# ztlpn/minilp

Measured on AMD Instinct MI355X. Metric: simplex pivots/sec, higher is better.
Workload: dtype f64; 1 GPU; config 4: random LP 100000 vars x 100000 constraints, 100 nnz/row (0.1% fill), Max c'x, Ax<=b, x>=0; primal simplex with PSE+DSE from the slack basis; timed pivots 5..1983; parallelism=1 GPU, nucleus_size_at_end=1559, completed_steps=1978

## Files before the change

minilp_amd/csrc/engine.h:

```cpp
#pragma once
#include <hip/hip_runtime.h>

#include <cstdint>
#include <functional>
#include <utility>
#include <stdexcept>
#include <string>
#include <vector>

#include "kernels.h"

namespace mlp {

enum Stage { STAGE_FTRAN = 0, STAGE_RATIO = 1, STAGE_BTRAN = 2, STAGE_BASIS = 3, STAGE_ROW = 4, STAGE_APPLY = 5 };

struct MlpError : std::runtime_error {
    int code;
    MlpError(int c, const std::string& s) : std::runtime_error(s), code(c) {}
};
struct LpFail {
    int code;
};

#define HIPCHECK(expr)                                                                                   \
// ... 109 lines not shown
    double fold_bytes = 0, fold_ms = 0;
    uint64_t fold_launches = 0;
    uint64_t kase[5] = {0, 0, 0, 0, 0};
};

enum class IterForm : int { Plain, PrimalHead, SmallBasis, MediumRide, LargeRide, ShardedPull, Factor };
enum class FtranEntry : int { Fused, GatherLrh, PrepGather };
enum class RowForm : int { Inside, Sparse, Sweep };
struct IterPlan {
    int phase, pse, dse, lazy, wtau, inl, fac;
    IterForm form;
    FtranEntry ftran;
    int ftran_ys, ftran_fpk;
    int tk_ride, rk_inside;
    int v_ride;
    int btran, btran_rhs;
    int sb_tk_inside;
    int post_touch, post_rk_ride;
    int basis_lists_touched;
    RowForm row;
    int row_lists;
    int pull_inside, with_struct;
    int fac_fused, fac_rho_part, fac_pair;
};

class Engine {
public:
    Engine();
    ~Engine();
    Engine(const Engine&) = delete;
// ... 420 lines not shown
```

minilp_amd/csrc/engine.hip:

```cpp
#include "engine.h"


#include <algorithm>
#include <chrono>
#include <cmath>
#include <cstdio>
#include <cstdlib>
#include <climits>
#include <cstring>
#include <limits>
#include <map>
#include <memory>
#include <mutex>

#include <dlfcn.h>
#include <fcntl.h>
#include <sys/mman.h>
#include <sys/stat.h>
#include <unistd.h>

namespace mlp {

static const double INF = std::numeric_limits<double>::infinity();
static double now_s() {
// ... 1310 lines not shown
    const bool fpl_base = g.fp && phase == 0 && pse && lazy && !stepping && !smallb && !g.head_fused && max_col_nnz_ <= HEAD_LIST_CAP && fpull_supported(dv, g);
    const bool fpl = fpl_base && ((tkr && ftran_head_rides_gather(dv, g)) || (shard_world > 1 && dv.lrJ > 0 && dv.pb_on && !dv.det_pull && dv.rowinfo != nullptr));
    const bool btr = !phead && !smallb && !tkr && !fpl && phase == 0 && pse && lazy && !stepping && shard_world == 1 && !shard_is_live() && btran_rides_ratio(dv, g);
    pl.form = phead ? IterForm::PrimalHead : smallb ? IterForm::SmallBasis : btr ? IterForm::MediumRide : tkr ? IterForm::LargeRide
              : fpl ? IterForm::ShardedPull : IterForm::Plain;
    if (phase == 0 && g.head_fused) pl.ftran = FtranEntry::Fused;
    else if (phase == 0 && !stepping && max_col_nnz_ <= HEAD_LIST_CAP && (fpl || ftran_head_rides_gather(dv, g))) pl.ftran = FtranEntry::GatherLrh;
    else pl.ftran = FtranEntry::PrepGather;
    pl.ftran_ys = tkr ? 1 : 0, pl.ftran_fpk = fpl ? 1 : 0;
    pl.tk_ride = tkr ? 1 : ((tkr_s || btr) ? 2 : 0), pl.rk_inside = btr ? 1 : 0;
    pl.btran = (phead || smallb || rkr || btr) ? 0 : 1;
    pl.btran_rhs = (phase == 0 && !tkr && !fpl) ? pse : 0;
    pl.sb_tk_inside = tkr_s ? 0 : 1;
    pl.post_touch = (g.str && phase == 0) ? 1 : 0, pl.post_rk_ride = rkr ? 1 : 0;
    pl.v_ride = (btr && !pl.post_touch && v_rides_ratio(dv, g)) ? 1 : 0;
    pl.basis_lists_touched = (phead || smallb || post_fused_lists_touched(dv, g, pse, 0, pl.post_touch)) ? 1 : 0;
    pl.pull_inside = (phead && g.str && update_pulls_inside(dv, g)) ? (head_applies(dv, g) ? 2 : 1) : 0;
    pl.row = !g.str ? RowForm::Sweep : (pl.pull_inside ? RowForm::Inside : RowForm::Sparse);
    pl.row_lists = (phase == 1 && !g.str && sweep_lists(dv, 0, 1)) ? 1 : 0;
    pl.with_struct = (phase == 1 && !pse) ? 1 : 0;
    return pl;
}
void Engine::launch_stage(const IterPlan& pl, int stage, bool with_events) {
    const DevView& dv = hview;
    const Geom g = geom();
    const int phase = pl.phase, pse = pl.pse;
    const bool phead = pl.form == IterForm::PrimalHead;
    if (phead && (stage == STAGE_RATIO || stage == STAGE_BTRAN || stage == STAGE_BASIS)) return;
    const bool fused = pl.fac_fused, pair = pl.fac_pair;
    const int dse = pl.dse, rho_whole = pl.fac_rho_part ? 0 : 8;
// ... 50 lines not shown
        break;
    case STAGE_BASIS:
        if (pl.fac) {
            if (pse && !(phase == 0 && pair)) launch_fac_solve(dv, g, 1, 1, 1, nullptr, 0, st);
            if (dse && !(phase == 1 && pair)) launch_fac_solve(dv, g, 0, 1, 1, nullptr, 0, st);
            break;
        }
        if (pl.form == IterForm::SmallBasis) {
            time_slot(2, 2);
            launch_small_basis(dv, g, st, pl.sb_tk_inside);
            time_slot(2, -1);
            break;
        }
        if (pl.v_ride) {
            time_slot(2, 2);
            launch_eta_vtail(dv, g, st);
            time_slot(2, -1);
            break;
        }
        time_slot(2, 2), time_slot(3, 10);
        launch_fused_w(dv, g, pse, st, pl.wtau);
        time_slot(2, -1), time_slot(3, -1);
        launch_post_fused(dv, g, pse, st, 0, 0, pl.wtau, pl.post_touch, pl.post_rk_ride);
        break;
    case STAGE_ROW:
        if (pl.row == RowForm::Inside) stamp(0), stamp(1);
        else if (pl.row == RowForm::Sparse) {
            stamp(0);
            if (phase == 0) launch_row_sparse(dv, g, pse, phead ? 0 : 1, pl.basis_lists_touched ? 0 : 1, st);
            else launch_row_sparse(dv, g, 0, 0, 1, st);
            stamp(1);
        } else {
            if (!pl.fac) time_slot(1, 0);
            if (phase == 0) launch_sweep(dv, g, pse, pl.fac ? 0 : 1, st, pl.inl);
            else launch_sweep(dv, g, 0, 0, st, 0, 1);
            if (!pl.fac) time_slot(1, -1);
        }
        break;
    case STAGE_APPLY:
        if (phase == 1 && pse) {
            if (pl.row == RowForm::Sparse) launch_row_sparse(dv, g, 2, 1, 0, st);
            else launch_sweep(dv, g, 2, pl.fac ? 0 : 1, st);
        }
        stamp(4);
        if (pl.fac && !fused) launch_fac_append(dv, st);
        launch_update_pivot(dv, g, phase, dse, pse, st, pl.inl, pl.with_struct, pl.pull_inside);
        stamp(5);
        break;
    default:
        throw MlpError(-1, "unknown stage");
    }
}
static bool use_graph_env() {
    const char* ng = std::getenv("MLP_NO_GRAPH");
    return !(ng && ng[0] == '1');
}
void Engine::record_iteration(const IterPlan& pl, bool with_events) {
    if (with_events) HIPCHECK(hipEventRecord(ev[8], st));
    static const bool debug_sync = std::getenv("MLP_DEBUG_SYNC") != nullptr && !use_graph_env();
    for (int i = 0; i < 6; ++i) {
        launch_stage(pl, kStageOrder[pl.phase][i], with_events);
// ... 1834 lines not shown
        tmp = {(double)n_, (double)p_};
    } else if (w == "fpull") {
        tmp = {(double)(hview.fpk_on ? 1 : 0), (double)fpk_builds_, (double)fpk_built_at_, (double)(fpull_supported(hview, geom()) ? 1 : 0)};
    } else if (w == "ratio_primal_form") {
        tmp = {(double)ratio_primal_form(hview, geom())};
    } else if (w == "ratio_list") {
        pull_ctl();
        const Geom g_ = geom();
        tmp = {(double)((ratio_primal_form(hview, g_) == 1 && ratio_list_cap(hview, g_) >= 0) ? 1 : 0), (double)h_ctl->rl_decisions, (double)h_ctl->rl_overflows};
    } else if (w == "btran_ride") {
        pull_ctl();
        tmp = {(double)(btran_rides_ratio(hview, geom()) ? 1 : 0), (double)h_ctl->rk_rides};
    } else if (w == "v_ride") {
        pull_ctl();
        tmp = {(double)(v_rides_ratio(hview, geom()) ? 1 : 0), (double)h_ctl->v_rides};
    } else if (w == "golive_checks") {
        tmp = {(double)golive_checks_};
    } else if (w == "shard_live") {
        tmp = {(double)(shard_is_live() ? 1 : 0)};
    } else if (w == "primal_head_launches") {
        pull_ctl();
        tmp = {(double)h_ctl->ph_count};
    }
    else if (w == "hyper_profile") {
        pull_ctl();
        for (int i = 0; i < 13; ++i) tmp.push_back((double)h_ctl->hy_prof[i] * 0.01);
        tmp.push_back((double)h_ctl->hy_prof[13]);
        tmp.push_back((double)h_ctl->hy_prof[14] * 0.01);
        tmp.push_back(0.0);
        for (int i = 16; i < 24; ++i) tmp.push_back((double)h_ctl->hy_prof[i] * 0.01);
// ... 945 lines not shown
```

minilp_amd/csrc/kernels.h:

```cpp
#pragma once
#include <hip/hip_runtime.h>
#include <stdint.h>

namespace mlp {

constexpr double EPS = 1e-8;

enum IterStatus : int {
    ITER_PIVOT = 0,
    ITER_FLIP = 1,
    ITER_OPTIMAL = 2,
    ITER_UNBOUNDED = 3,
    ITER_FEASIBLE = 4,
    ITER_INFEASIBLE = 5,
    ITER_SINGULAR = 6,
    ITER_NONE = 7,
    ITER_COMM = 8,
    ITER_STALL = 9,
};

struct IterState {
    int status;
    int q;
    int r;
// ... 66 lines not shown
    int ph_count;
    int ph_rng_x, ph_rng_y;
    int ar_used;
    int ar_n;
    int rv_n;
    unsigned long long hy_prof[24];
    PivotRec ring[RING];
    int ar_off;
    int ar_back;
    int ar_pauses;
    int ar_keep;
    int rk_rides;
    int rl_decisions;
    int rl_overflows;
    int v_rides;
};

constexpr int MAIL_KINDS = 6;
constexpr int MAX_WORLD = 16;
struct alignas(64) MailRec {
    unsigned long long epoch;
    double f[7];
};

constexpr uint8_t NB_AT_MIN = 1, NB_AT_MAX = 2, NB_FIXED = 4;
__host__ __device__ inline int nb_status_of(uint8_t f) {
    if ((f & NB_FIXED) || ((f & NB_AT_MIN) && (f & NB_AT_MAX))) return 4;
    return (f & NB_AT_MIN) ? 1 : ((f & NB_AT_MAX) ? 2 : 3);
}

// ... 165 lines not shown
    int* fac_brow;
    int* fac_bslot_of_row;
    double* fac_Wb;
    const FacSbRec* fac_sb_rec; const int* fac_sb_lptr; const int* fac_sb_oidx; const double* fac_sb_oval;
    const int* fac_sb_trow; const int* fac_sb_tcol; const double* fac_sb_tinv; const double* fac_sb_tinvT;
};
constexpr int FAC_BMAX = 1024;
constexpr int AR_CAP = 2048;
constexpr int RK_LDS = 64;
constexpr int RL_CAP = 8;
constexpr int RL_BLOCKS = 512;
constexpr int TK_ONE = 128;
constexpr int TK_GROUPS = 16;
constexpr int TK_STRIDE = 1024;
constexpr int TK_WORDS = TK_STRIDE * (TK_GROUPS + 1) + 8;
constexpr int FAC_BAR_FLAG = TK_WORDS + 1024;

constexpr int FW_TR = 8;
constexpr int FW_TC = 1024;

constexpr int BAND_ROWS = 8192;
constexpr int BAND_THREADS = 1024;
constexpr int PB_ROWS = 4096;
constexpr int PB_CHUNKS = 48;
constexpr int PB_CHUNKS_DEFAULT = 24;

struct Geom {
    int m, n, cap;
    int lanes;
    int sweep_one;
// ... 17 lines not shown
void launch_price_dual(const DevView& dv, const Geom& g, int use_dse, hipStream_t st);
void launch_ftran_prep(const DevView& dv, int derive_primal, hipStream_t st);
void launch_ftran_gather(const DevView& dv, const Geom& g, hipStream_t st, int ys = 0);
void launch_ftran_fused(const DevView& dv, const Geom& g, int derive_primal, hipStream_t st);
bool ftran_head_rides_gather(const DevView& dv, const Geom& g);
void launch_ftran_gather_lrh(const DevView& dv, const Geom& g, hipStream_t st, int ys = 0, int fpk = 0);
bool fpull_supported(const DevView& dv, const Geom& g);
void launch_fpull_ratio(const DevView& dv, const Geom& g, hipStream_t st, hipEvent_t ftran_done = nullptr);
void launch_fpk_build(const DevView& dv, hipStream_t st);
void launch_btran_fused(const DevView& dv, const Geom& g, int with_rhs, int derive_dual, hipStream_t st);
constexpr int HEAD_LIST_CAP = 1024;
void launch_ratio_primal(const DevView& dv, const Geom& g, int use_pse, hipStream_t st, int tk_ride = 0, int rk_inside = 0, int v_ride = 0);
bool tk_rides_ratio(const DevView& dv, const Geom& g);
bool btran_rides_ratio(const DevView& dv, const Geom& g);
bool v_rides_ratio(const DevView& dv, const Geom& g);
void launch_eta_vtail(const DevView& dv, const Geom& g, hipStream_t st);
int ratio_list_cap(const DevView& dv, const Geom& g);
int ratio_primal_form(const DevView& dv, const Geom& g);
bool tk_rides_ratio_small(const DevView& dv, const Geom& g);
void launch_post_ftran(const DevView& dv, const Geom& g, int use_pse, hipStream_t st);
void launch_btran_prep(const DevView& dv, int derive_dual, int plan_after, hipStream_t st);
void launch_btran(const DevView& dv, const Geom& g, int with_rhs, hipStream_t st, int after_fold = 0);
void launch_btran_rhs(const DevView& dv, const Geom& g, hipStream_t st);
void launch_sweep(const DevView& dv, const Geom& g, int mode, int with_struct, hipStream_t st, int inline_combine = 0, int list = 0);
void launch_row_sparse(const DevView& dv, const Geom& g, int mode, int with_struct, int touch, hipStream_t st);
bool small_basis_supported(const DevView& dv, const Geom& g);
void launch_small_basis(const DevView& dv, const Geom& g, hipStream_t st, int tk_inside = 1);
bool primal_head_supported(const DevView& dv, const Geom& g);
int primal_head_kmax(int longest_column);
void launch_primal_head(const DevView& dv, hipStream_t st, int list, int applies);
void launch_init_nb_rng(const DevView& dv, const Geom& g, hipStream_t st);
void launch_ratio_dual(const DevView& dv, const Geom& g, hipStream_t st, int list_ok = 0);
void launch_fused_w(const DevView& dv, const Geom& g, int with_v, hipStream_t st, int with_tau = 1);
void launch_post_fused(const DevView& dv, const Geom& g, int with_v, hipStream_t st, int classic = 0, int skip_push = 0, int with_tau = 1, int touch = 0, int rk_ride = 0);
bool rk_rides_post(const DevView& dv, const Geom& g);
void launch_exact_beta(const DevView& dv, hipStream_t st);
void launch_hyper_dual(const DevView& dv, int use_dse, int max_iters, long heavy, hipStream_t st);
void launch_mail_handshake(const DevView& dv, int* out, hipStream_t st);
constexpr int MAIL_PUMP_RECS = MAIL_KINDS * 2 + 1;
void launch_mail_stage(const DevView& dv, void* stage, hipStream_t st);
void launch_mail_deliver(const DevView& dv, const void* stage, hipStream_t st);
void arm_kernel_timing(int slot, hipEvent_t t0, hipEvent_t t1);
bool fold_fuses_v(const DevView& dv, int with_v, int with_tau, int fold_only);
int stream_coresident_blocks();
void launch_structure_update(const DevView& dv, const Geom& g, hipStream_t st);
void launch_update_pivot(const DevView& dv, const Geom& g, int phase, int use_dse, int use_pse, hipStream_t st, int inline_comb = 0,
                         int with_struct = 0, int pull_inside = 0);
bool update_pulls_inside(const DevView& dv, const Geom& g);
bool head_applies(const DevView& dv, const Geom& g);
void launch_set_iter(const DevView& dv, int status, int q, int r, double lnv, int forced, hipStream_t st);
void launch_reset_ring(const DevView& dv, hipStream_t st);
void launch_btran_dense(const DevView& dv, const Geom& g, hipStream_t st);
void launch_recalc_d(const DevView& dv, const Geom& g, hipStream_t st);
void launch_recalc_basic_vals(const DevView& dv, const Geom& g, const double* rhs, double* r_tmp, int refine, hipStream_t st);
void launch_shift_nonbasic(const DevView& dv, const Geom& g, int col, double val, hipStream_t st);
void launch_sq_norms_add_row(const DevView& dv, const Geom& g, hipStream_t st);
void launch_copy_rho_sq_to_beta(const DevView& dv, int row, hipStream_t st);
void launch_build_nucleus(const DevView& dv, const Geom& g, double* Kd, int k, hipStream_t st);
void launch_fac_solve(const DevView& dv, const Geom& g, int dir, int src, int dst, const double* src_ptr, int always, hipStream_t st, int fuse = 0);
void launch_fac_solve2(const DevView& dv, const Geom& g, int dir, int srcA, int dstA, int srcB, int dstB, hipStream_t st, int fuse = 0);
void fac_solve_set_sharers(int n);
int fac_solve_grid_blocks();
// ... 159 lines not shown
```

minilp_amd/csrc/kernels.hip:

```cpp
#include "kernels.h"
#include <hip/hip_ext.h>

#include <limits.h>
#include <math.h>

#include <cstdlib>
#include <string>

namespace mlp {

#define NONE_IDX INT_MAX
constexpr int BLK = 256;

struct Cand {
    double key;
    int idx;
};
__device__ __forceinline__ Cand cand_none() { return Cand{-INFINITY, NONE_IDX}; }
__device__ __forceinline__ bool cand_better(const Cand& a, const Cand& b) {
    return a.key > b.key || (a.key == b.key && a.idx < b.idx);
}
__device__ __forceinline__ Cand wave_best(Cand c) {
#pragma unroll
    for (int o = 32; o > 0; o >>= 1) {
// ... 157 lines not shown
        s_key[w] = c.key;
        s_idx[w] = c.idx;
        s_pay[w] = pay;
    }
    __syncthreads();
    if (threadIdx.x == 0) {
        for (int i = 1; i < BLK / 64; ++i) {
            Cand t{s_key[i], s_idx[i]};
            if (cand_better(t, c)) {
                c = t;
                pay = s_pay[i];
            }
        }
    }
}
__device__ __forceinline__ bool grid_best_p(Cand& c, double& pay, const DevView& v, int nblocks = -1) {
    if (nblocks < 0) nblocks = (int)gridDim.x;
    block_best_p(c, pay);
    if (threadIdx.x == 0) {
        st_agent(&v.red_key[blockIdx.x], c.key);
        st_agent(&v.red_idx[blockIdx.x], c.idx);
        st_agent(&v.red_key2[blockIdx.x], pay);
    }
    if (!last_block_arrives(v.ticket, (unsigned)nblocks)) return false;
    KMARK(v.ctl, 16);
    Cand x = cand_none();
    double xp = 0.0;
    for (int i = threadIdx.x; i < nblocks; i += blockDim.x) {
        Cand t{ld_agent(&v.red_key[i]), ld_agent(&v.red_idx[i])};
        if (cand_better(t, x)) {
            x = t;
            xp = ld_agent(&v.red_key2[i]);
        }
    }
    KMARK(v.ctl, 17);
    block_best_p(x, xp);
    c = x;
    pay = xp;
    if (threadIdx.x == 0) *v.ticket = 0;
// ... 47 lines not shown
}
#define LAUNCH_T(slot, kern, grid, block, lds, st, ...)                                                          \
    do {                                                                                                         \
        if (g_tev[slot][0]) hipExtLaunchKernelGGL(kern, grid, block, lds, st, g_tev[slot][0], g_tev[slot][1], 0, __VA_ARGS__); \
        else hipLaunchKernelGGL(kern, grid, block, lds, st, __VA_ARGS__);                                        \
    } while (0)
static inline int blocks_for(long n, int per_block = BLK) { return n <= 0 ? 1 : (int)((n + per_block - 1) / per_block); }

template <int G>
__device__ __forceinline__ double group_sum(double x) {
#pragma unroll
    for (int o = G / 2; o > 0; o >>= 1) x += __shfl_xor(x, o, 64);
    return x;
}

__device__ __forceinline__ void push_rec(Ctl* c, int phase) {
    int n = c->ring_n;
    if (n < RING) {
        PivotRec& r = c->ring[n];
        r.status = c->it.status;
        r.phase = phase;
        r.q = c->it.q;
        r.r = c->it.r;
        r.entering_var = c->it.entering_var;
        r.leaving_var = c->it.leaving_var;
        r.kase = c->up.kase;
        r.k_after = c->k;
        r.klist_n = c->it.klist_n;
        r.blist_n = c->it.blist_n;
        r.pivot_coeff = c->it.pivot_coeff;
        if (c->kprof_on == 2) r.pivot_coeff = c->it.alpha_sq;
        else if (c->kprof_on == 3) r.pivot_coeff = c->it.rho_sq;
        else if (c->kprof_on == 4) r.pivot_coeff = c->it.inv_alpha;
        else if (c->kprof_on == 5) {
            double sh = 0.0;
            for (int j = 0; j < c->nlow && j < LR_MAX; ++j) sh += c->lr_h[j];
            r.pivot_coeff = sh;
        }
        r.obj = c->it.obj;
    }
    c->ring_n = n + 1;
}
// ... 498 lines not shown
        it->q = -1;
        it->r = -1;
        c->halt = 1;
        push_rec(c, phase);
    } else {
        it->status = ITER_PIVOT;
        if (phase == 0) {
            it->q = best.idx;
            it->r = -1;
        } else {
            it->r = best.idx;
            it->q = -1;
        }
    }
}
__device__ __forceinline__ void close_and_open(const DevView& v, Ctl* c, int phase, Cand best, double pay, bool close_current) {
    __shared__ double s_key, s_pay;
    __shared__ int s_idx, s_go;
    if (threadIdx.x == 0) {
        if (close_current) push_rec(c, phase);
        if (close_current && v.str_on) {
            c->hyper_epoch += 1;
            c->str_n = 0;
            c->aq_n = 0;
        }
        s_go = 1;
        if (close_current && c->forced) {
            c->halt = 1;
            s_go = 0;
        }
        s_key = best.key;
        s_idx = best.idx;
        s_pay = pay;
    }
    __syncthreads();
// ... 1624 lines not shown
            v.Ut[(size_t)kold * LR_MAX + s] = 0.0;
            v.V[(size_t)s * ld + kold] = 0.0;
        }
    } else if (u.kase == 3) {
        if (s < kold) {
            const double un = -v.aK[s] * inv_alpha;
            Un[s] = un;
            v.Ut[(size_t)s * LR_MAX + jn] = un;
            Vn[s] = (s == u.cq) ? 0.0 : v.rK[s];
        }
        if (s < jn) v.V[(size_t)s * ld + u.cq] = 0.0;
    }
    if (s == 0) c->nlow = jn + 1;
}
__device__ __forceinline__ void fpk_append_wave(const DevView& v, const Ctl* c, int lane);
__device__ __forceinline__ void struct_update_body(const DevView& v, Ctl* c, int s) {
    const StructUpdate u = c->up;
    if (u.kase < 0) return;
    if (v.fpk_on && s < 64) fpk_append_wave(v, c, s);
    if (v.lrJ) lowrank_append(v, c, u, s);
    if (u.kase == 0) return;
    const int kold = u.kold;
    const int ld = v.ld;
    const double inv_alpha = c->it.inv_alpha;
    if (u.kase == 1) {
        if (s < kold) {
            v.W[(size_t)kold * ld + s] = v.rK[s] * inv_alpha;
            v.W[(size_t)s * ld + kold] = -v.aK[s] * u.inv_diag_r * inv_alpha;
        } else if (s == kold) {
            v.W[(size_t)kold * ld + kold] = u.inv_diag_r * inv_alpha;
            v.kslot_of_pos[u.r] = kold;
            v.pos_of_kslot[kold] = u.r;
            v.kslot_of_row[u.i_r] = kold;
            v.rowinfo[u.i_r] = RowInfo{0.0, -1, kold};
            v.row_of_kslot[kold] = u.i_r;
            c->k = kold + 1;
        }
    } else if (u.kase == 2) {
        const int last = kold - 1;
        if (s < last) {
            if (u.sr != last) v.W[(size_t)u.sr * ld + s] = v.W[(size_t)last * ld + (s == u.cq ? last : s)];
            if (u.cq != last) v.W[(size_t)s * ld + u.cq] = v.W[(size_t)(s == u.sr ? last : s) * ld + last];
        }
        if (s == 0) {
            if (u.sr != last) {
                int pl = v.pos_of_kslot[last];
                v.pos_of_kslot[u.sr] = pl;
                v.kslot_of_pos[pl] = u.sr;
            }
            v.kslot_of_pos[u.r] = -1;
            v.srow_of_pos[u.r] = u.i_q;
            v.sdiag_of_pos[u.r] = u.diag_q;
            if (u.cq != last) {
                int il = v.row_of_kslot[last];
                v.row_of_kslot[u.cq] = il;
                v.kslot_of_row[il] = u.cq;
                v.rowinfo[il] = RowInfo{0.0, -1, u.cq};
            }
            v.kslot_of_row[u.i_q] = -1;
            v.pos_of_srow[u.i_q] = u.r;
            v.rowinfo[u.i_q] = RowInfo{u.diag_q, u.r, -1};
            c->k = last;
        }
    } else if (u.kase == 3) {
        if (s < kold) v.W[(size_t)s * ld + u.cq] = -v.aK[s] * u.inv_diag_r * inv_alpha;
        if (s == 0) {
            v.srow_of_pos[u.r] = u.i_q;
            v.sdiag_of_pos[u.r] = u.diag_q;
            v.kslot_of_row[u.i_q] = -1;
            v.pos_of_srow[u.i_q] = u.r;
            v.rowinfo[u.i_q] = RowInfo{u.diag_q, u.r, -1};
            v.kslot_of_row[u.i_r] = u.cq;
            v.rowinfo[u.i_r] = RowInfo{0.0, -1, u.cq};
            v.row_of_kslot[u.cq] = u.i_r;
        }
    } else if (u.kase == 4) {
        if (s == 0) {
            v.sdiag_of_pos[u.r] = u.diag_q;
            v.rowinfo[v.srow_of_pos[u.r]] = RowInfo{u.diag_q, u.r, -1};
        }
// ... 519 lines not shown
    if (NT) {
        dbl2_t t = __builtin_nontemporal_load(reinterpret_cast<const dbl2_t*>(p));
        return make_double2(t.x, t.y);
    }
    return *reinterpret_cast<const double2*>(p);
}
template <bool NT>
__device__ __forceinline__ void fw_store2(double* p, double a, double b) {
    if (NT) {
        dbl2_t t = {a, b};
        __builtin_nontemporal_store(t, reinterpret_cast<dbl2_t*>(p));
    } else {
        *reinterpret_cast<double2*>(p) = make_double2(a, b);
    }
}
template <int TR, int TC>
__device__ __forceinline__ void v_tail_body(const DevView& v, const Ctl* c, int b, int k, int fold_fused, bool xsh, const double* xb);
template <int TR, bool WITH_TAU, bool WITH_V, bool DO_UPDATE, bool NT = false, bool LR = false, int RL = 1, bool TILED = false, bool VT = false>
__global__ void __launch_bounds__(BLK) k_fused_w(DevView v) {
    static_assert(!VT || (TR == 8 && !WITH_TAU && !WITH_V && DO_UPDATE && !LR && !TILED), "the v tail rides with the eta-only pass of 8-row tiles");
    Ctl* c = v.ctl;
    if (c->halt || c->it.status != ITER_PIVOT) return;
    KMARK0(c, 8);
    if (LR && c->fold) return;
    const int k = c->k, ld = v.ld;
    if (VT && blockIdx.y == 0) {
        if (blockIdx.x == 0 && threadIdx.x == 0) atomicAdd(&c->v_rides, 1);
        v_tail_body<TR, FW_TC>(v, c, (int)blockIdx.x, k, 0, false, nullptr);
        return;
    }
// ... 31 lines not shown
    cidx[1] = cidx[0] + 1;
    cidx[2] = col0 + 512 + 2 * tid;
    cidx[3] = cidx[2] + 1;
    double rk[4];
#pragma unroll
    for (int j = 0; j < 4; ++j) rk[j] = (cidx[j] < k) ? v.rK[cidx[j]] : 0.0;
    const double inv_alpha = DO_UPDATE ? c->it.inv_alpha : 0.0;
    const int rslot = DO_UPDATE ? c->up.sr : -1;
    double vacc[4] = {0.0, 0.0, 0.0, 0.0};
    const bool pair0 = cidx[1] < k, pair1 = cidx[3] < k;
    const bool one0 = cidx[0] < k, one1 = cidx[2] < k;
    const int wv = tid >> 6, l = tid & 63;
#pragma unroll 1
    for (int sub = 0; sub < RL; ++sub) {
        double tacc[TR];
        if constexpr (DO_UPDATE) {
            constexpr int GR = 8;
            const int c0 = one0 ? cidx[0] : col0, c2 = one1 ? cidx[2] : col0;
#pragma unroll
            for (int g0 = 0; g0 < TR; g0 += GR) {
                double2 wa[GR], wb[GR];
                double tk[GR], ak[GR];
#pragma unroll
                for (int a = 0; a < GR; ++a) {
                    const int row = row0 + sub * TR + g0 + a;
                    const int rc = row < k ? row : k - 1;
                    const double* wp = v.W + (size_t)rc * ld;
                    wa[a] = fw_load2<NT>(wp + c0);
                    wb[a] = fw_load2<NT>(wp + c2);
                    tk[a] = WITH_V ? v.tK[rc] : 0.0;
                    ak[a] = v.aK[rc];
// ... 570 lines not shown
    }
}
template <int TR>
__global__ void __launch_bounds__(BLK) k_reduce_v(DevView v) {
    Ctl* c = v.ctl;
    const int k = c->k;
    int i = blockIdx.x * BLK + threadIdx.x;
    if (i >= k) return;
    const int nstripes = (k + TR - 1) / TR;
    double s = 0.0;
    for (int t = 0; t < nstripes; ++t) s += v.part_v[(size_t)t * v.ld + i];
    v.vK[i] = s;
    v.rv[v.row_of_kslot[i]].y = s;
}

__global__ void __launch_bounds__(BLK) k_update_pivot(DevView v, int phase, int use_dse, int use_pse, int inline_comb, int n_upd, int pull_inside) {
    Ctl* c = v.ctl;
    if (c->halt) return;
    const IterState* it = &c->it;
    const int status = it->status;
    if (status != ITER_PIVOT && status != ITER_FLIP) return;
    KMARK0(c, 12);
    if ((int)blockIdx.x >= n_upd) {
        if (status == ITER_PIVOT)
            struct_update_body(v, c, ((int)blockIdx.x - n_upd) * BLK + threadIdx.x);
        return;
    }
    const bool flip = status == ITER_FLIP;
    const int r = flip ? -1 : it->r, q = it->q;
    const double pc = it->pivot_coeff;
    constexpr int UPT = 4;
    __shared__ int s_tl[BLK * UPT];
    __shared__ double s_ta[BLK * UPT], s_th[BLK * UPT];
    __shared__ int s_tcnt;
    int my_slot[UPT] = {-1, -1, -1, -1};
    double pre_d[UPT] = {0.0, 0.0, 0.0, 0.0}, pre_g[UPT] = {1.0, 1.0, 1.0, 1.0};
    uint8_t pre_f[UPT] = {0, 0, 0, 0};
    const bool pre = pull_inside && !flip;
    if (pull_inside) {
        if (threadIdx.x == 0) s_tcnt = 0;
// ... 185 lines not shown
                    }
                    if (v.str_on && !pull_inside) v.alpha_r[tn] = 0.0;
                }
            }
            if (phase == 0 && tn >= v.nb_lo && tn < v.nb_hi) {
                tc = price_primal_one(dd, gm, f, tn, use_pse);
                tc_d = dd;
            }
        }
        if (cand_better(tc, cand)) {
            cand = tc;
            cand_d = tc_d;
        }
    }
    KMARK0(c, 13);
    if (!grid_best_p(cand, cand_d, v, n_upd)) return;
    KMARK(c, 14);
    close_and_open(v, c, phase, cand, cand_d, true);
    KMARK(c, 15);
}

__global__ void k_set_iter(DevView v, int status, int q, int r, double lnv, int forced) {
    Ctl* c = v.ctl;
    IterState* it = &c->it;
    it->status = status;
    it->q = q;
    it->r = r;
    it->leaving_new_val = lnv;
    it->entering_var = q >= 0 ? v.nb_vars[q] : -1;
    it->leaving_var = r >= 0 ? v.basic_vars[r] : -1;
    it->klist_n = 0;
    it->blist_n = 0;
    c->up.kase = -1;
// ... 975 lines not shown
    dim3 gr(nstripes, nchunks), b(BLK);
    if (rows == 8) {
        if (with_v && with_tau) LAUNCH_T(2, (k_fused_w<8, true, true, true>), gr, b, 0, st, dv);
        else if (with_v) LAUNCH_T(2, (k_fused_w<8, false, true, true>), gr, b, 0, st, dv);
        else if (with_tau) LAUNCH_T(2, (k_fused_w<8, true, false, true>), gr, b, 0, st, dv);
        else LAUNCH_T(2, (k_fused_w<8, false, false, true>), gr, b, 0, st, dv);
    } else {
        const long tiles_cap = (long)nstripes * nchunks;
        const int nb = (int)(tiles_cap < FW_TILE_BLOCKS ? tiles_cap : FW_TILE_BLOCKS);
        if (with_v && with_tau) LAUNCH_T(2, (k_fused_w<16, true, true, true, true, false, 1, true>), dim3(nb), b, 0, st, dv);
        else if (with_v) LAUNCH_T(2, (k_fused_w<16, false, true, true, true, false, 1, true>), dim3(nb), b, 0, st, dv);
        else if (with_tau) LAUNCH_T(2, (k_fused_w<16, true, false, true, true, false, 1, true>), dim3(nb), b, 0, st, dv);
        else LAUNCH_T(2, (k_fused_w<16, false, false, true, true, false, 1, true>), dim3(nb), b, 0, st, dv);
    }
}
void launch_eta_vtail(const DevView& dv, const Geom& g, hipStream_t st) {
    if (g.cap <= 0) return;
    const int nstripes = (g.cap + 8 - 1) / 8, nchunks = (g.cap + FW_TC - 1) / FW_TC;
    LAUNCH_T(2, (k_fused_w<8, false, false, true, false, false, 1, false, true>), dim3(nstripes, nchunks + 1), dim3(BLK), 0, st, dv);
}
bool rk_rides_post(const DevView& dv, const Geom& g) {
    const char* e = std::getenv("MLP_RK_RIDE");
    if (e && e[0] == '0') return false;
    return strip_tiled(dv, g) && !dv.wshard && dv.world <= 1;
}
void launch_post_fused(const DevView& dv, const Geom& g, int with_v, hipStream_t st, int classic, int skip_push, int with_tau, int touch, int rk_ride) {
    if (!with_tau) skip_push = 1;
    if (!with_tau && !with_v) return;
    if (!classic && strip_tiled(dv, g)) {
        if (dv.wshard) hipLaunchKernelGGL((k_post_exchange<STRIP_RB, STRIP_CH>), dim3(blocks_for(g.cap)), dim3(BLK), 0, st, dv, with_v, with_tau);
#define POSTS(G)                                                                                                  \
    do {                                                                                                          \
        int n_push = with_tau ? blocks_for((long)g.cap * G) : 0;                                                  \
        if (with_v && rk_ride) {                                                                                  \
// ... 29 lines not shown
void launch_structure_update(const DevView& dv, const Geom& g, hipStream_t st) {
    hipLaunchKernelGGL(k_struct_update, dim3(blocks_for(g.cap)), dim3(BLK), 0, st, dv);
}
bool update_pulls_inside(const DevView& dv, const Geom& g) {
    const char* e = std::getenv("MLP_PULL_INSIDE");
    if (e && e[0] == '0') return false;
    const int t = g.m > g.n ? g.m : g.n;
    return primal_head_supported(dv, g) && blocks_for(t, BLK * 4) <= 2048 && dv.hy_stamp_n != nullptr;
}
bool head_applies(const DevView& dv, const Geom& g) {
    const char* e = std::getenv("MLP_HEAD_APPLY");
    if (e && e[0] == '0') return false;
    return update_pulls_inside(dv, g) && dv.nb_order == nullptr && dv.pk_valid == nullptr;
}
void launch_update_pivot(const DevView& dv, const Geom& g, int phase, int use_dse, int use_pse, hipStream_t st, int inline_comb,
                         int with_struct, int pull_inside) {
    int t = g.m > g.n ? g.m : g.n;
    const int upd_pt = std::max(1, std::min(8, (blocks_for(t) + 511) / 512));
    int n_upd = blocks_for(t, BLK * upd_pt) <= 2048 ? blocks_for(t, BLK * upd_pt) : 2048;
    const int pull_pt = std::max(1, std::min(4, (blocks_for(pull_inside == 2 ? g.n : t) + 511) / 512));
    if (pull_inside == 2) n_upd = blocks_for(g.n, BLK * pull_pt);
    else if (pull_inside) n_upd = blocks_for(t, BLK * pull_pt);
    hipLaunchKernelGGL(k_update_pivot, dim3(n_upd + (with_struct ? blocks_for(g.cap) : 0)), dim3(BLK), 0, st, dv, phase, use_dse, use_pse,
                       inline_comb, n_upd, pull_inside);
}
void launch_set_iter(const DevView& dv, int status, int q, int r, double lnv, int forced, hipStream_t st) {
    hipLaunchKernelGGL(k_set_iter, dim3(1), dim3(1), 0, st, dv, status, q, r, lnv, forced);
}
void launch_reset_ring(const DevView& dv, hipStream_t st) { hipLaunchKernelGGL(k_reset_ring, dim3(1), dim3(1), 0, st, dv); }
void launch_btran_dense(const DevView& dv, const Geom& g, hipStream_t st) {
    if (dv.fac_on) {
        launch_fac_gather_cb(dv, st);
        launch_fac_solve(dv, g, 1, 2, 1, dv.alpha_q, 1, st);
        return;
    }
    if (g.cap <= 0) return;
    hipLaunchKernelGGL(k_gather_basic_obj, dim3(blocks_for(g.m)), dim3(BLK), 0, st, dv);
    launch_btran_rhs(dv, g, st);
    int nstripes = (g.cap + 16 - 1) / 16, nchunks = (g.cap + FW_TC - 1) / FW_TC;
// ... 108 lines not shown
```

Baseline: 12150 pivots/s.

## Fold eta W-update and structure update into the pivot-update kernel

When the v tail rides the ratio kernel, the eta rank-1 update of the dense W inverse moves out of the eta_vtail launch into extra blocks of k_update_pivot. Those blocks also apply the permutation and column fix-ups, meet on a second ticket, then run the structure update (skipping the W writes already done) and join the grid reduction as a guest arrival. The eta_vtail launch then covers only the tail, and the sweep stops doing the separate structure update. This removes a dependent launch and overlaps the W update with the pivot update, but it adds a two-level ticket handshake and extra blocks to the update kernel, plus tricky index handling for the case-2 row and column moves.

After: 11930 pivots/s. 1.8% lower.

```diff
diff --git a/minilp_amd/csrc/engine.h b/minilp_amd/csrc/engine.h
--- a/minilp_amd/csrc/engine.h
+++ b/minilp_amd/csrc/engine.h
@@ -147,6 +147,8 @@
     int ftran_ys, ftran_fpk;
     int tk_ride, rk_inside;
     int v_ride;
+    int eta_ride;
+    int sweep_struct;
     int btran, btran_rhs;
     int sb_tk_inside;
     int post_touch, post_rk_ride;
diff --git a/minilp_amd/csrc/engine.hip b/minilp_amd/csrc/engine.hip
--- a/minilp_amd/csrc/engine.hip
+++ b/minilp_amd/csrc/engine.hip
@@ -1348,6 +1348,8 @@
     pl.sb_tk_inside = tkr_s ? 0 : 1;
     pl.post_touch = (g.str && phase == 0) ? 1 : 0, pl.post_rk_ride = rkr ? 1 : 0;
     pl.v_ride = (btr && !pl.post_touch && v_rides_ratio(dv, g)) ? 1 : 0;
+    pl.eta_ride = (pl.v_ride && eta_rides_update(dv, g)) ? 1 : 0;
+    pl.sweep_struct = (pl.fac || pl.eta_ride) ? 0 : 1;
     pl.basis_lists_touched = (phead || smallb || post_fused_lists_touched(dv, g, pse, 0, pl.post_touch)) ? 1 : 0;
     pl.pull_inside = (phead && g.str && update_pulls_inside(dv, g)) ? (head_applies(dv, g) ? 2 : 1) : 0;
     pl.row = !g.str ? RowForm::Sweep : (pl.pull_inside ? RowForm::Inside : RowForm::Sparse);
@@ -1428,7 +1430,7 @@
         }
         if (pl.v_ride) {
             time_slot(2, 2);
-            launch_eta_vtail(dv, g, st);
+            launch_eta_vtail(dv, g, st, pl.eta_ride);
             time_slot(2, -1);
             break;
         }
@@ -1446,7 +1448,7 @@
             stamp(1);
         } else {
             if (!pl.fac) time_slot(1, 0);
-            if (phase == 0) launch_sweep(dv, g, pse, pl.fac ? 0 : 1, st, pl.inl);
+            if (phase == 0) launch_sweep(dv, g, pse, pl.sweep_struct, st, pl.inl);
             else launch_sweep(dv, g, 0, 0, st, 0, 1);
             if (!pl.fac) time_slot(1, -1);
         }
@@ -1458,7 +1460,7 @@
         }
         stamp(4);
         if (pl.fac && !fused) launch_fac_append(dv, st);
-        launch_update_pivot(dv, g, phase, dse, pse, st, pl.inl, pl.with_struct, pl.pull_inside);
+        launch_update_pivot(dv, g, phase, dse, pse, st, pl.inl, pl.with_struct, pl.pull_inside, pl.eta_ride);
         stamp(5);
         break;
     default:
@@ -3323,6 +3325,9 @@
     } else if (w == "v_ride") {
         pull_ctl();
         tmp = {(double)(v_rides_ratio(hview, geom()) ? 1 : 0), (double)h_ctl->v_rides};
+    } else if (w == "eta_ride") {
+        pull_ctl();
+        tmp = {(double)(eta_rides_update(hview, geom()) ? 1 : 0), (double)h_ctl->eta_rides};
     } else if (w == "golive_checks") {
         tmp = {(double)golive_checks_};
     } else if (w == "shard_live") {
diff --git a/minilp_amd/csrc/kernels.h b/minilp_amd/csrc/kernels.h
--- a/minilp_amd/csrc/kernels.h
+++ b/minilp_amd/csrc/kernels.h
@@ -104,6 +104,7 @@
     int rl_decisions;
     int rl_overflows;
     int v_rides;
+    int eta_rides;
 };
 
 constexpr int MAIL_KINDS = 6;
@@ -299,6 +300,8 @@
 constexpr int TK_GROUPS = 16;
 constexpr int TK_STRIDE = 1024;
 constexpr int TK_WORDS = TK_STRIDE * (TK_GROUPS + 1) + 8;
+constexpr int TK_SECOND = 32;
+static_assert(TK_SECOND + TK_STRIDE * TK_GROUPS < TK_WORDS, "the second ticket's first-step tickets lie inside the buffer");
 constexpr int FAC_BAR_FLAG = TK_WORDS + 1024;
 
 constexpr int FW_TR = 8;
@@ -346,7 +349,8 @@
 bool tk_rides_ratio(const DevView& dv, const Geom& g);
 bool btran_rides_ratio(const DevView& dv, const Geom& g);
 bool v_rides_ratio(const DevView& dv, const Geom& g);
-void launch_eta_vtail(const DevView& dv, const Geom& g, hipStream_t st);
+void launch_eta_vtail(const DevView& dv, const Geom& g, hipStream_t st, int tail_only = 0);
+bool eta_rides_update(const DevView& dv, const Geom& g);
 int ratio_list_cap(const DevView& dv, const Geom& g);
 int ratio_primal_form(const DevView& dv, const Geom& g);
 bool tk_rides_ratio_small(const DevView& dv, const Geom& g);
@@ -377,7 +381,7 @@
 int stream_coresident_blocks();
 void launch_structure_update(const DevView& dv, const Geom& g, hipStream_t st);
 void launch_update_pivot(const DevView& dv, const Geom& g, int phase, int use_dse, int use_pse, hipStream_t st, int inline_comb = 0,
-                         int with_struct = 0, int pull_inside = 0);
+                         int with_struct = 0, int pull_inside = 0, int eta_ride = 0);
 bool update_pulls_inside(const DevView& dv, const Geom& g);
 bool head_applies(const DevView& dv, const Geom& g);
 void launch_set_iter(const DevView& dv, int status, int q, int r, double lnv, int forced, hipStream_t st);
diff --git a/minilp_amd/csrc/kernels.hip b/minilp_amd/csrc/kernels.hip
--- a/minilp_amd/csrc/kernels.hip
+++ b/minilp_amd/csrc/kernels.hip
@@ -195,15 +195,18 @@
         }
     }
 }
-__device__ __forceinline__ bool grid_best_p(Cand& c, double& pay, const DevView& v, int nblocks = -1) {
+__device__ __forceinline__ bool grid_best_p(Cand& c, double& pay, const DevView& v, int nblocks = -1, int n_arrive = -1, bool guest = false, int my = -1) {
     if (nblocks < 0) nblocks = (int)gridDim.x;
-    block_best_p(c, pay);
-    if (threadIdx.x == 0) {
-        st_agent(&v.red_key[blockIdx.x], c.key);
-        st_agent(&v.red_idx[blockIdx.x], c.idx);
-        st_agent(&v.red_key2[blockIdx.x], pay);
-    }
-    if (!last_block_arrives(v.ticket, (unsigned)nblocks)) return false;
+    if (n_arrive < 0) n_arrive = nblocks;
+    if (!guest) {
+        block_best_p(c, pay);
+        if (threadIdx.x == 0) {
+            st_agent(&v.red_key[blockIdx.x], c.key);
+            st_agent(&v.red_idx[blockIdx.x], c.idx);
+            st_agent(&v.red_key2[blockIdx.x], pay);
+        }
+    }
+    if (!last_block_arrives(v.ticket, (unsigned)n_arrive, guest ? my : -1)) return false;
     KMARK(v.ctl, 16);
     Cand x = cand_none();
     double xp = 0.0;
@@ -281,7 +284,7 @@
     return x;
 }
 
-__device__ __forceinline__ void push_rec(Ctl* c, int phase) {
+__device__ __forceinline__ void push_rec(Ctl* c, int phase, bool k_planned = false) {
     int n = c->ring_n;
     if (n < RING) {
         PivotRec& r = c->ring[n];
@@ -293,6 +296,7 @@
         r.leaving_var = c->it.leaving_var;
         r.kase = c->up.kase;
         r.k_after = c->k;
+        if (k_planned && c->up.kase >= 0) r.k_after = c->up.kold + (c->up.kase == 1 ? 1 : (c->up.kase == 2 ? -1 : 0));
         r.klist_n = c->it.klist_n;
         r.blist_n = c->it.blist_n;
         r.pivot_coeff = c->it.pivot_coeff;
@@ -821,11 +825,11 @@
         }
     }
 }
-__device__ __forceinline__ void close_and_open(const DevView& v, Ctl* c, int phase, Cand best, double pay, bool close_current) {
+__device__ __forceinline__ void close_and_open(const DevView& v, Ctl* c, int phase, Cand best, double pay, bool close_current, bool k_planned = false) {
     __shared__ double s_key, s_pay;
     __shared__ int s_idx, s_go;
     if (threadIdx.x == 0) {
-        if (close_current) push_rec(c, phase);
+        if (close_current) push_rec(c, phase, k_planned);
         if (close_current && v.str_on) {
             c->hyper_epoch += 1;
             c->str_n = 0;
@@ -2480,7 +2484,7 @@
     if (s == 0) c->nlow = jn + 1;
 }
 __device__ __forceinline__ void fpk_append_wave(const DevView& v, const Ctl* c, int lane);
-__device__ __forceinline__ void struct_update_body(const DevView& v, Ctl* c, int s) {
+__device__ __forceinline__ void struct_update_body(const DevView& v, Ctl* c, int s, bool w_done = false) {
     const StructUpdate u = c->up;
     if (u.kase < 0) return;
     if (v.fpk_on && s < 64) fpk_append_wave(v, c, s);
@@ -2491,6 +2495,7 @@
     const double inv_alpha = c->it.inv_alpha;
     if (u.kase == 1) {
         if (s < kold) {
+            if (w_done) return;
             v.W[(size_t)kold * ld + s] = v.rK[s] * inv_alpha;
             v.W[(size_t)s * ld + kold] = -v.aK[s] * u.inv_diag_r * inv_alpha;
         } else if (s == kold) {
@@ -2504,7 +2509,7 @@
         }
     } else if (u.kase == 2) {
         const int last = kold - 1;
-        if (s < last) {
+        if (s < last && !w_done) {
             if (u.sr != last) v.W[(size_t)u.sr * ld + s] = v.W[(size_t)last * ld + (s == u.cq ? last : s)];
             if (u.cq != last) v.W[(size_t)s * ld + u.cq] = v.W[(size_t)(s == u.sr ? last : s) * ld + last];
         }
@@ -2529,7 +2534,7 @@
             c->k = last;
         }
     } else if (u.kase == 3) {
-        if (s < kold) v.W[(size_t)s * ld + u.cq] = -v.aK[s] * u.inv_diag_r * inv_alpha;
+        if (s < kold && !w_done) v.W[(size_t)s * ld + u.cq] = -v.aK[s] * u.inv_diag_r * inv_alpha;
         if (s == 0) {
             v.srow_of_pos[u.r] = u.i_q;
             v.sdiag_of_pos[u.r] = u.diag_q;
@@ -3079,6 +3084,89 @@
         *reinterpret_cast<double2*>(p) = make_double2(a, b);
     }
 }
+template <bool NT, bool PC = false>
+__device__ __forceinline__ void eta_rows8(const DevView& v, int k, int ld, int rowbase, int col0, const int (&cidx)[4], const double (&rk)[4],
+                                          double inv_alpha, int rslot, const StructUpdate* pu = nullptr) {
+    const bool pair0 = cidx[1] < k, pair1 = cidx[3] < k;
+    const bool one0 = cidx[0] < k, one1 = cidx[2] < k;
+    const int c0 = one0 ? cidx[0] : col0, c2 = one1 ? cidx[2] : col0;
+    const int kase = PC ? pu->kase : 0, last = k - 1;
+    const int ks = (PC && kase == 2) ? last : k;
+    const int cq = (PC && (kase == 2 || kase == 3)) ? pu->cq : -1;
+    int jq = -1;
+#pragma unroll
+    for (int j = 0; j < 4; ++j)
+        if (PC && cidx[j] == cq) jq = j;
+    const bool mv_row = PC && kase == 2 && rslot != last && rslot >= rowbase && rslot < rowbase + 8;
+    const bool mv_col = PC && kase == 2 && cq != last && jq >= 0;
+    double2 wa[8], wb[8];
+    double ak[8];
+#pragma unroll
+    for (int a = 0; a < 8; ++a) {
+        const int row = rowbase + a;
+        const int rc = row < k ? row : k - 1;
+        const double* wp = v.W + (size_t)rc * ld;
+        wa[a] = fw_load2<NT>(wp + c0);
+        wb[a] = fw_load2<NT>(wp + c2);
+        ak[a] = v.aK[rc];
+    }
+    double2 la = make_double2(0.0, 0.0), lb = make_double2(0.0, 0.0);
+    double ak_l = 0.0, w_ll = 0.0, rk_l = 0.0, wl[8] = {0.0, 0.0, 0.0, 0.0, 0.0, 0.0, 0.0, 0.0};
+    if (PC) {
+        if (mv_row) {
+            const double* wp = v.W + (size_t)last * ld;
+            la = fw_load2<NT>(wp + c0);
+            lb = fw_load2<NT>(wp + c2);
+            ak_l = v.aK[last];
+            if (jq >= 0) w_ll = wp[last];
+        }
+        if (mv_col) {
+#pragma unroll
+            for (int a = 0; a < 8; ++a) {
+                const int row = rowbase + a;
+                wl[a] = v.W[(size_t)(row < k ? row : k - 1) * ld + last];
+            }
+        }
+        if ((mv_row && jq >= 0) || mv_col) rk_l = v.rK[last];
+    }
+#pragma unroll
+    for (int a = 0; a < 8; ++a) {
+        const int row = rowbase + a;
+        if (row >= ks) continue;
+        double* wp = v.W + (size_t)row * ld;
+        double w[4] = {one0 ? wa[a].x : 0.0, pair0 ? wa[a].y : 0.0, one1 ? wb[a].x : 0.0, pair1 ? wb[a].y : 0.0};
+        const double u = (ak[a] - (row == rslot ? 1.0 : 0.0)) * inv_alpha;
+#pragma unroll
+        for (int j = 0; j < 4; ++j) w[j] -= u * rk[j];
+        if (PC) {
+            if (kase == 3) {
+                const double t = -ak[a] * pu->inv_diag_r * inv_alpha;
+#pragma unroll
+                for (int j = 0; j < 4; ++j)
+                    if (j == jq) w[j] = t;
+            } else if (mv_row && row == rslot) {
+                const double ul = (ak_l - 0.0) * inv_alpha;
+                double e[4] = {one0 ? la.x : 0.0, pair0 ? la.y : 0.0, one1 ? lb.x : 0.0, pair1 ? lb.y : 0.0};
+#pragma unroll
+                for (int j = 0; j < 4; ++j) {
+                    e[j] -= ul * rk[j];
+                    if (j == jq) e[j] = w_ll - ul * rk_l;
+                    w[j] = e[j];
+                }
+            } else if (mv_col) {
+                const double t = wl[a] - u * rk_l;
+#pragma unroll
+                for (int j = 0; j < 4; ++j)
+                    if (j == jq) w[j] = t;
+            }
+        }
+        const bool sp0 = cidx[1] < ks, sp1 = cidx[3] < ks, so0 = cidx[0] < ks, so1 = cidx[2] < ks;
+        if (sp0) fw_store2<NT>(wp + cidx[0], w[0], w[1]);
+        else if (so0) wp[cidx[0]] = w[0];
+        if (sp1) fw_store2<NT>(wp + cidx[2], w[2], w[3]);
+        else if (so1) wp[cidx[2]] = w[2];
+    }
+}
 template <int TR, int TC>
 __device__ __forceinline__ void v_tail_body(const DevView& v, const Ctl* c, int b, int k, int fold_fused, bool xsh, const double* xb);
 template <int TR, bool WITH_TAU, bool WITH_V, bool DO_UPDATE, bool NT = false, bool LR = false, int RL = 1, bool TILED = false, bool VT = false>
@@ -3140,7 +3228,9 @@
 #pragma unroll 1
     for (int sub = 0; sub < RL; ++sub) {
         double tacc[TR];
-        if constexpr (DO_UPDATE) {
+        if constexpr (DO_UPDATE && TR == 8 && !WITH_TAU && !WITH_V) {
+            eta_rows8<NT, false>(v, k, ld, row0 + sub * TR, col0, cidx, rk, inv_alpha, rslot);
+        } else if constexpr (DO_UPDATE) {
             constexpr int GR = 8;
             const int c0 = one0 ? cidx[0] : col0, c2 = one1 ? cidx[2] : col0;
 #pragma unroll
@@ -3741,16 +3831,66 @@
     v.rv[v.row_of_kslot[i]].y = s;
 }
 
-__global__ void __launch_bounds__(BLK) k_update_pivot(DevView v, int phase, int use_dse, int use_pse, int inline_comb, int n_upd, int pull_inside) {
+__device__ __forceinline__ bool eta_rider(const DevView& v, Ctl* c, int rb, int eta_ns, int eta_nt) {
+    const int k = c->k, ld = v.ld, tid = threadIdx.x;
+    const int stripe = rb % eta_ns, chunk = rb / eta_ns;
+    const int row0 = stripe * 8, col0 = chunk * FW_TC;
+    if (row0 < k && col0 < k) {
+        const StructUpdate u = c->up;
+        const double inv_alpha = c->it.inv_alpha;
+        int cidx[4];
+        cidx[0] = col0 + 2 * tid;
+        cidx[1] = cidx[0] + 1;
+        cidx[2] = col0 + 512 + 2 * tid;
+        cidx[3] = cidx[2] + 1;
+        double rk[4];
+#pragma unroll
+        for (int j = 0; j < 4; ++j) rk[j] = (cidx[j] < k) ? v.rK[cidx[j]] : 0.0;
+        const double ak_new = (u.kase == 1 && col0 == 0 && tid < 8 && row0 + tid < k) ? v.aK[row0 + tid] : 0.0;
+        eta_rows8<false, true>(v, k, ld, row0, col0, cidx, rk, inv_alpha, u.sr, &u);
+        if (u.kase == 1) {
+            if (row0 == 0) {
+                double* wp = v.W + (size_t)k * ld;
+                if (cidx[1] < k) *reinterpret_cast<double2*>(wp + cidx[0]) = make_double2(rk[0] * inv_alpha, rk[1] * inv_alpha);
+                else if (cidx[0] < k) wp[cidx[0]] = rk[0] * inv_alpha;
+                if (cidx[3] < k) *reinterpret_cast<double2*>(wp + cidx[2]) = make_double2(rk[2] * inv_alpha, rk[3] * inv_alpha);
+                else if (cidx[2] < k) wp[cidx[2]] = rk[2] * inv_alpha;
+            }
+            if (col0 == 0 && tid < 8 && row0 + tid < k) v.W[(size_t)(row0 + tid) * ld + k] = -ak_new * u.inv_diag_r * inv_alpha;
+        }
+    }
+    __syncthreads();
+    if (!last_block_arrives(v.ticket + TK_SECOND, (unsigned)eta_nt, rb)) return false;
+    if (tid == 0) {
+        v.ticket[TK_SECOND] = 0;
+        atomicAdd(&c->eta_rides, 1);
+    }
+    const int lim = max(c->up.kold, 63);
+    for (int s = tid; s <= lim; s += BLK) struct_update_body(v, c, s, true);
+    KMARK(c, 23);
+    return true;
+}
+__global__ void __launch_bounds__(BLK) k_update_pivot(DevView v, int phase, int use_dse, int use_pse, int inline_comb, int n_upd, int pull_inside,
+                                                      int eta_ns, int eta_nt) {
     Ctl* c = v.ctl;
     if (c->halt) return;
     const IterState* it = &c->it;
     const int status = it->status;
     if (status != ITER_PIVOT && status != ITER_FLIP) return;
     KMARK0(c, 12);
+    const int n_arrive = n_upd + ((eta_ns > 0 && status == ITER_PIVOT) ? 1 : 0);
     if ((int)blockIdx.x >= n_upd) {
-        if (status == ITER_PIVOT)
-            struct_update_body(v, c, ((int)blockIdx.x - n_upd) * BLK + threadIdx.x);
+        if (eta_ns > 0) {
+            if (status != ITER_PIVOT || !eta_rider(v, c, (int)blockIdx.x - n_upd, eta_ns, eta_nt)) return;
+            Cand none = cand_none();
+            double none_d = 0.0;
+            if (!grid_best_p(none, none_d, v, n_upd, n_arrive, true, n_upd)) return;
+            KMARK(c, 14);
+            close_and_open(v, c, phase, none, none_d, true, true);
+            KMARK(c, 15);
+            return;
+        }
+        if (status == ITER_PIVOT) struct_update_body(v, c, ((int)blockIdx.x - n_upd) * BLK + threadIdx.x);
         return;
     }
     const bool flip = status == ITER_FLIP;
@@ -3966,9 +4106,9 @@
         }
     }
     KMARK0(c, 13);
-    if (!grid_best_p(cand, cand_d, v, n_upd)) return;
+    if (!grid_best_p(cand, cand_d, v, n_upd, n_arrive)) return;
     KMARK(c, 14);
-    close_and_open(v, c, phase, cand, cand_d, true);
+    close_and_open(v, c, phase, cand, cand_d, true, n_arrive > n_upd);
     KMARK(c, 15);
 }
 
@@ -4974,10 +5114,16 @@
         else LAUNCH_T(2, (k_fused_w<16, false, false, true, true, false, 1, true>), dim3(nb), b, 0, st, dv);
     }
 }
-void launch_eta_vtail(const DevView& dv, const Geom& g, hipStream_t st) {
+void launch_eta_vtail(const DevView& dv, const Geom& g, hipStream_t st, int tail_only) {
     if (g.cap <= 0) return;
     const int nstripes = (g.cap + 8 - 1) / 8, nchunks = (g.cap + FW_TC - 1) / FW_TC;
-    LAUNCH_T(2, (k_fused_w<8, false, false, true, false, false, 1, false, true>), dim3(nstripes, nchunks + 1), dim3(BLK), 0, st, dv);
+    const dim3 gr = tail_only ? dim3(blocks_for(g.cap, 32), 1) : dim3(nstripes, nchunks + 1);
+    LAUNCH_T(2, (k_fused_w<8, false, false, true, false, false, 1, false, true>), gr, dim3(BLK), 0, st, dv);
+}
+bool eta_rides_update(const DevView& dv, const Geom& g) {
+    const char* e = std::getenv("MLP_ETA_RIDE");
+    if (e && e[0] == '0') return false;
+    return v_rides_ratio(dv, g);
 }
 bool rk_rides_post(const DevView& dv, const Geom& g) {
     const char* e = std::getenv("MLP_RK_RIDE");
@@ -5037,15 +5183,16 @@
     return update_pulls_inside(dv, g) && dv.nb_order == nullptr && dv.pk_valid == nullptr;
 }
 void launch_update_pivot(const DevView& dv, const Geom& g, int phase, int use_dse, int use_pse, hipStream_t st, int inline_comb,
-                         int with_struct, int pull_inside) {
+                         int with_struct, int pull_inside, int eta_ride) {
     int t = g.m > g.n ? g.m : g.n;
+    const int eta_ns = eta_ride ? (g.cap + 8 - 1) / 8 : 0, eta_nt = eta_ns * ((g.cap + FW_TC - 1) / FW_TC);
     const int upd_pt = std::max(1, std::min(8, (blocks_for(t) + 511) / 512));
     int n_upd = blocks_for(t, BLK * upd_pt) <= 2048 ? blocks_for(t, BLK * upd_pt) : 2048;
     const int pull_pt = std::max(1, std::min(4, (blocks_for(pull_inside == 2 ? g.n : t) + 511) / 512));
     if (pull_inside == 2) n_upd = blocks_for(g.n, BLK * pull_pt);
     else if (pull_inside) n_upd = blocks_for(t, BLK * pull_pt);
-    hipLaunchKernelGGL(k_update_pivot, dim3(n_upd + (with_struct ? blocks_for(g.cap) : 0)), dim3(BLK), 0, st, dv, phase, use_dse, use_pse,
-                       inline_comb, n_upd, pull_inside);
+    hipLaunchKernelGGL(k_update_pivot, dim3(n_upd + (eta_ride ? eta_nt : (with_struct ? blocks_for(g.cap) : 0))), dim3(BLK), 0, st, dv, phase, use_dse,
+                       use_pse, inline_comb, n_upd, pull_inside, eta_ns, eta_nt);
 }
 void launch_set_iter(const DevView& dv, int status, int q, int r, double lnv, int forced, hipStream_t st) {
     hipLaunchKernelGGL(k_set_iter, dim3(1), dim3(1), 0, st, dv, status, q, r, lnv, forced);
```
